# neoyinyao/Recommender

Measured on AMD Instinct MI355X. Metric: examples/sec fwd+bwd, Criteo-DLRM 26×40M×128 batch 65536, 1/2/4/8 GPU, higher is better.
Workload: dtype fp32; 1 GPU; dlrm_criteo_26x40000000x128; global_batch=65536, per_gpu_batch=65536, rows=40000000, dim=128, slots=26, optimizer=sgd, parallelism=single, prefetch=False

## Files before the change

recommender_amd/csrc/sort.hip:

```cpp
#include "common.hpp"

namespace rs {

constexpr int kSortThreads = 256;
constexpr int kSortKeysPerLane = 16;
constexpr int kSortTile = kSortThreads * kSortKeysPerLane;
constexpr int kSortKeysPerLaneSmall = 4;
constexpr int kSortKeysPerLaneTiny = 2;
constexpr int64_t kSortSmallN = 1 << 20;
constexpr int64_t kSortTinyN = 1 << 17;
static inline int sort_kpl(int64_t n) {
  return n < kSortTinyN ? kSortKeysPerLaneTiny : (n < kSortSmallN ? kSortKeysPerLaneSmall : kSortKeysPerLane);
}
constexpr int kMaxBins = 512;

template <int BITS>
__device__ __forceinline__ uint64_t match_digit(uint32_t digit, bool valid) {
  uint32_t mis_lo = 0u, mis_hi = 0u;
#pragma unroll
  for (int b = 0; b < BITS; ++b) {
    const uint32_t sgn = (uint32_t)(-(int32_t)((digit >> b) & 1u));
    const uint64_t bb = __ballot(sgn != 0u);
    mis_lo |= (uint32_t)bb ^ sgn;
    mis_hi |= (uint32_t)(bb >> 32) ^ sgn;
// ... 338 lines not shown
    flags[i] = (k < key_space && (i == 0 || keys[i - 1] != k)) ? 1 : 0;
  }
}

__global__ void unique_inverse_kernel(const uint32_t* __restrict__ keys, const int32_t* __restrict__ pos,
                                      const int32_t* __restrict__ excl, int64_t n, uint32_t key_space,
                                      uint32_t* __restrict__ uniq, int32_t* __restrict__ inverse) {
  int64_t i = blockIdx.x * (int64_t)blockDim.x + threadIdx.x;
  int64_t stride = (int64_t)gridDim.x * blockDim.x;
  for (; i < n; i += stride) {
    const uint32_t k = keys[i];
    const bool valid = k < key_space;
    const bool head = valid && (i == 0 || keys[i - 1] != k);
    const int32_t seg = excl[i] + (head ? 1 : 0) - 1;
    if (head) uniq[seg] = k;
    inverse[pos[i]] = valid ? seg : -1;
  }
}

__global__ void owner_counts_kernel(const uint32_t* __restrict__ uniq, const int32_t* __restrict__ n_unique,
                                    int64_t shard_stride, int32_t world, int32_t* __restrict__ counts) {
  const int o = threadIdx.x;
  if (o >= world) return;
  const int32_t nu = *n_unique;
  auto lb = [&](int64_t v) {
    int32_t lo = 0, hi = nu;
    while (lo < hi) {
      int32_t mid = (lo + hi) >> 1;
      if ((int64_t)uniq[mid] < v) lo = mid + 1; else hi = mid;
    }
    return lo;
  };
  counts[o] = lb((int64_t)(o + 1) * shard_stride) - lb((int64_t)o * shard_stride);
}

static int key_bits_for(int64_t n_rows) {
  int b = 1;
  while (b < 32 && ((int64_t)1 << b) <= n_rows) ++b;
  return b;
}

struct SortPlan {
  int passes;
  int bits;
  int kpl;
  int n_tiles;
};

static SortPlan plan_sort(int64_t n_ids, int64_t n_rows) {
  SortPlan p;
  int kb = key_bits_for(n_rows);
  p.passes = (kb + 8) / 9;
  p.bits = (kb + p.passes - 1) / p.passes;
  p.kpl = sort_kpl(n_ids);
  p.n_tiles = (int)ceil_div(n_ids, (int64_t)kSortThreads * p.kpl);
  return p;
}

static size_t sort_ws_layout(int64_t n_ids, Carver& c, uint32_t** keys_alt, int32_t** vals_alt,
                             int32_t** hist, int32_t** totals) {
  int n_tiles = (int)ceil_div(n_ids, (int64_t)kSortThreads * sort_kpl(n_ids));
  *keys_alt = c.take<uint32_t>(n_ids);
  *vals_alt = c.take<int32_t>(n_ids);
  *hist = c.take<int32_t>((size_t)kMaxBins * n_tiles + 1);
  *totals = c.take<int32_t>(kMaxBins);
  return c.off;
}

template <int BITS, bool FIRST_FROM_IDS, int KPL>
static int32_t launch_pass_k(uint32_t* kin, const int32_t* vin, uint32_t* kout, int32_t* vout,
                             int64_t n, int shift, int32_t* hist, int32_t* totals, int n_tiles,
                             const KeyGen& kg, hipStream_t st, uint32_t clamp_key) {
  radix_hist_kernel<BITS, FIRST_FROM_IDS, KPL><<<n_tiles, kSortThreads, 0, st>>>(kin, kg, n, shift,
                                                                                 hist, n_tiles);
  RS_CHECK_LAUNCH();
  constexpr int BINS = 1 << BITS;
  radix_colscan_kernel<<<(BINS + 3) / 4, 256, 0, st>>>(hist, n_tiles, BINS, totals);
  RS_CHECK_LAUNCH();
  radix_scatter_kernel<BITS, FIRST_FROM_IDS, KPL><<<n_tiles, kSortThreads, 0, st>>>(
      kin, vin, n, shift, hist, totals, n_tiles, kout, vout, clamp_key);
  RS_CHECK_LAUNCH();
  return RS_OK;
}

template <int BITS, bool FIRST_FROM_IDS>
static int32_t launch_pass(uint32_t* kin, const int32_t* vin, uint32_t* kout, int32_t* vout,
                           int64_t n, int shift, int32_t* hist, int32_t* totals, int n_tiles,
                           const KeyGen& kg, hipStream_t st, uint32_t clamp_key) {
  if (sort_kpl(n) == kSortKeysPerLaneTiny)
    return launch_pass_k<BITS, FIRST_FROM_IDS, kSortKeysPerLaneTiny>(kin, vin, kout, vout, n, shift,
                                                                     hist, totals, n_tiles, kg, st,
                                                                     clamp_key);
  if (sort_kpl(n) == kSortKeysPerLaneSmall)
    return launch_pass_k<BITS, FIRST_FROM_IDS, kSortKeysPerLaneSmall>(kin, vin, kout, vout, n, shift,
                                                                      hist, totals, n_tiles, kg, st,
                                                                      clamp_key);
  return launch_pass_k<BITS, FIRST_FROM_IDS, kSortKeysPerLane>(kin, vin, kout, vout, n, shift, hist,
                                                               totals, n_tiles, kg, st, clamp_key);
}

template <bool FIRST_FROM_IDS>
static int32_t dispatch_pass(int bits, uint32_t* kin, const int32_t* vin, uint32_t* kout,
                             int32_t* vout, int64_t n, int shift, int32_t* hist, int32_t* totals,
                             int n_tiles, const KeyGen& kg, hipStream_t st, uint32_t clamp_key) {
#define RS_PASS(B) \
  case B: return launch_pass<B, FIRST_FROM_IDS>(kin, vin, kout, vout, n, shift, hist, totals, n_tiles, kg, st, clamp_key);
  switch (bits) {
    RS_PASS(1) RS_PASS(2) RS_PASS(3) RS_PASS(4) RS_PASS(5) RS_PASS(6) RS_PASS(7) RS_PASS(8) RS_PASS(9)
  }
#undef RS_PASS
  set_error("radix pass bits %d unsupported", bits);
  return RS_E_UNSUPPORTED;
}

static int32_t radix_sort_impl(uint32_t* keys_in, int32_t* vals_in, uint32_t* keys_out,
                               int32_t* vals_out, int64_t n, int64_t max_key, void* ws,
                               size_t ws_bytes, const KeyGen* kg, hipStream_t st) {
  SortPlan p = plan_sort(n, max_key);
  Carver c(ws, ws_bytes);
  uint32_t* kalt;
  int32_t* valt;
  int32_t* hist;
  int32_t* totals;
  sort_ws_layout(n, c, &kalt, &valt, &hist, &totals);
  if (!c.ok()) {
    set_error("sort workspace too small: need %zu have %zu", c.off, ws_bytes);
    return RS_E_WORKSPACE;
  }
  uint32_t* ka = keys_in;
  int32_t* va = vals_in;
  const KeyGen none{};
  for (int pass = 0; pass < p.passes; ++pass) {
    bool last = pass == p.passes - 1;
    uint32_t* kb = last ? keys_out : (ka == keys_in ? kalt : keys_in);
    int32_t* vb = last ? vals_out : (va == vals_in ? valt : vals_in);
    const uint32_t clamp = (last && kg) ? static_cast<uint32_t>(kg->key_space) : 0xFFFFFFFFu;
    int32_t s = (pass == 0 && kg)
                    ? dispatch_pass<true>(p.bits, ka, va, kb, vb, n, 0, hist, totals, p.n_tiles, *kg, st,
                                          clamp)
                    : dispatch_pass<false>(p.bits, ka, va, kb, vb, n, pass * p.bits, hist, totals,
                                           p.n_tiles, none, st, clamp);
    if (s) return s;
    ka = kb;
    va = vb;
  }
  return RS_OK;
}

int32_t radix_sort_pairs(uint32_t* keys_in, int32_t* vals_in, uint32_t* keys_out,
                         int32_t* vals_out, int64_t n, int64_t n_rows, void* ws, size_t ws_bytes,
                         hipStream_t st) {
  return radix_sort_impl(keys_in, vals_in, keys_out, vals_out, n, n_rows, ws, ws_bytes, nullptr, st);
}

size_t radix_sort_ws_size(int64_t n) {
  Carver c(nullptr, 0);
  uint32_t* a;
  int32_t* b;
  int32_t* h;
  int32_t* t;
  return sort_ws_layout(n, c, &a, &b, &h, &t) + 256;
}

__global__ __launch_bounds__(1024) void scan_single_block_kernel(int32_t* __restrict__ a, int64_t n,
                                                                 int32_t* __restrict__ total) {
  __shared__ int32_t wsum[16];
  __shared__ int32_t carry_s;
  const int t = threadIdx.x, lane = t & 63, w = t >> 6;
  if (t == 0) carry_s = 0;
  __syncthreads();
  for (int64_t base = 0; base < n; base += 4096) {
    int32_t v[4];
    int64_t i0 = base + (int64_t)t * 4;
#pragma unroll
    for (int k = 0; k < 4; ++k) v[k] = (i0 + k < n) ? a[i0 + k] : 0;
    int32_t s = v[0] + v[1] + v[2] + v[3];
    int32_t x = s;
#pragma unroll
    for (int off = 1; off < 64; off <<= 1) {
      int32_t y = __shfl_up(x, off);
      if (lane >= off) x += y;
    }
    if (lane == 63) wsum[w] = x;
    __syncthreads();
    if (t < 16) {
      int32_t ws = wsum[t];
      int32_t xs = ws;
#pragma unroll
      for (int off = 1; off < 16; off <<= 1) {
        int32_t y = __shfl_up(xs, off, 16);
        if ((t & 15) >= off) xs += y;
      }
      wsum[t] = xs - ws;
    }
    __syncthreads();
    int32_t run = carry_s + wsum[w] + x - s;
#pragma unroll
    for (int k = 0; k < 4; ++k) {
      if (i0 + k < n) a[i0 + k] = run;
      run += v[k];
    }
    __syncthreads();
    if (t == 1023) carry_s = run;
    __syncthreads();
  }
  if (t == 0 && total) *total = carry_s;
}

constexpr int kScanThreads = 256;
constexpr int kScanPerThread = 16;
constexpr int kScanTile = kScanThreads * kScanPerThread;

__global__ __launch_bounds__(kScanThreads) void scan_tile_sums_kernel(const int32_t* __restrict__ in,
                                                                      int64_t n,
                                                                      int32_t* __restrict__ sums) {
  __shared__ int32_t red[kScanThreads / 64];
  int64_t base = (int64_t)blockIdx.x * kScanTile;
  int32_t s = 0;
  int32_t v[kScanPerThread];
#pragma unroll
  for (int k = 0; k < kScanPerThread; ++k) {
    const int64_t i = base + (int64_t)k * kScanThreads + threadIdx.x;
    v[k] = in[i < n ? i : 0];
  }
#pragma unroll
  for (int k = 0; k < kScanPerThread; ++k)
    if (base + (int64_t)k * kScanThreads + threadIdx.x < n) s += v[k];
  for (int off = 32; off > 0; off >>= 1) s += __shfl_down(s, off);
  if ((threadIdx.x & 63) == 0) red[threadIdx.x >> 6] = s;
  __syncthreads();
  if (threadIdx.x == 0) {
    int32_t t = 0;
    for (int w = 0; w < kScanThreads / 64; ++w) t += red[w];
    sums[blockIdx.x] = t;
  }
}

__global__ __launch_bounds__(kScanThreads) void scan_tile_apply_kernel(const int32_t* __restrict__ in,
                                                                       int64_t n,
                                                                       const int32_t* __restrict__ sums,
                                                                       int32_t* __restrict__ out) {
  __shared__ int32_t part[kScanThreads];
  int64_t base = (int64_t)blockIdx.x * kScanTile + (int64_t)threadIdx.x * kScanPerThread;
  int32_t v[kScanPerThread];
  int32_t s = 0;
#pragma unroll
  for (int k = 0; k < kScanPerThread; ++k) {
    int64_t i = base + k;
    v[k] = i < n ? in[i] : 0;
    s += v[k];
  }
  part[threadIdx.x] = s;
  __syncthreads();
  for (int off = 1; off < kScanThreads; off <<= 1) {
    int32_t t = threadIdx.x >= off ? part[threadIdx.x - off] : 0;
    __syncthreads();
    part[threadIdx.x] += t;
    __syncthreads();
  }
  int32_t run = sums[blockIdx.x] + (threadIdx.x ? part[threadIdx.x - 1] : 0);
#pragma unroll
  for (int k = 0; k < kScanPerThread; ++k) {
    int64_t i = base + k;
    if (i < n) out[i] = run;
    run += v[k];
  }
}

size_t exclusive_scan_ws_size(int64_t n) { return align_up((ceil_div(n, kScanTile) + 1) * 4, 256); }

int32_t exclusive_scan_i32(const int32_t* in, int32_t* out, int64_t n, int32_t* total, void* ws,
                           size_t ws_bytes, hipStream_t st) {
  int64_t tiles = ceil_div(n, kScanTile);
  if (ws_bytes < exclusive_scan_ws_size(n)) {
    set_error("scan workspace too small");
    return RS_E_WORKSPACE;
  }
  int32_t* sums = static_cast<int32_t*>(ws);
  if (n == 0) {
    if (total) RS_CHECK_HIP(hipMemsetAsync(total, 0, 4, st));
    return RS_OK;
  }
  scan_tile_sums_kernel<<<tiles, kScanThreads, 0, st>>>(in, n, sums);
  RS_CHECK_LAUNCH();
  scan_single_block_kernel<<<1, 1024, 0, st>>>(sums, tiles, total);
  RS_CHECK_LAUNCH();
  scan_tile_apply_kernel<<<tiles, kScanThreads, 0, st>>>(in, n, sums, out);
  RS_CHECK_LAUNCH();
  return RS_OK;
}

constexpr int kSegThreads = 256;
#ifndef RS_SEG_KPL
#define RS_SEG_KPL 16
#endif
constexpr int kSegKPL = RS_SEG_KPL;
constexpr int kSegTile = kSegThreads * kSegKPL;
constexpr int kSegBits = 12;
constexpr int kSegBins = 1 << kSegBits;
constexpr int kSegMaxTiles = 32 * 16 / kSegKPL;
constexpr int kSegMaxSlots = 64;
constexpr int kSegMaxBits = 2 * kSegBits;
constexpr int kNumXcd = 8;

struct SegArgs {
  const void* ids;
  int32_t dtype;
  const uint8_t* valid;
  const int64_t* slot_offsets;
  int n_slots;
  int64_t B;
  int tiles;
  int64_t n_rows;
  uint16_t* hist0;
  uint16_t* hist1;
  int32_t* vcnt;
  int32_t* scnt;
  uint2* tmp;
  uint32_t* keys0;
  int32_t* starts;
  uint32_t* rows_out;
  int32_t* pos_out;
  int32_t* err_flag;
};

__device__ __forceinline__ int seg_bits(int64_t rows) {
  int b = 0;
  while (b < 31 && ((int64_t)1 << b) < rows) ++b;
  return b;
}

struct SegSlot {
  int64_t lo, rows;
  int w0, w1;
};

__device__ __forceinline__ SegSlot seg_slot(const SegArgs& a, int s) {
  SegSlot r;
  r.lo = a.slot_offsets ? a.slot_offsets[s] : 0;
  r.rows = a.slot_offsets ? a.slot_offsets[s + 1] - r.lo : a.n_rows;
  const int bits = seg_bits(r.rows);
  r.w0 = bits < kSegBits ? bits : kSegBits;
  r.w1 = bits - r.w0;
  if (r.w1 > kSegBits) {
    r.w1 = kSegBits;
    r.rows = (int64_t)1 << kSegMaxBits;
    if (threadIdx.x == 0 && a.err_flag) atomicOr(a.err_flag, RS_ERRBIT_RANGE);
  }
  return r;
}

__device__ __forceinline__ void seg_tile0(const SegArgs& a, int& s, int& t) {
  const int x = blockIdx.x % kNumXcd, rest = blockIdx.x / kNumXcd;
  s = rest % a.n_slots;
  t = (rest / a.n_slots) * kNumXcd + x;
}
__device__ __forceinline__ void seg_tile1(const SegArgs& a, int& s, int& t) {
  const int x = blockIdx.x % kNumXcd, rest = blockIdx.x / kNumXcd;
  const int spx = (a.n_slots + kNumXcd - 1) / kNumXcd;
  s = x + kNumXcd * (rest % spx);
  t = rest / spx;
}

template <bool ID64>
__device__ __forceinline__ void seg_load0(const SegArgs& a, const SegSlot& sl, int s, int t,
                                          uint32_t (&id)[kSegKPL], uint32_t& live,
                                          uint32_t& sent, bool& oob) {
  const int wave = threadIdx.x >> 6, lane = threadIdx.x & 63;
  int64_t v[kSegKPL];
  int64_t pp[kSegKPL];
  uint32_t inb = 0u;
#pragma unroll
  for (int k = 0; k < kSegKPL; ++k) {
    const int64_t b = (int64_t)t * kSegTile + wave * 64 * kSegKPL + k * 64 + lane;
    const bool in = b < a.B;
    inb |= (uint32_t)in << k;
    pp[k] = in ? b * a.n_slots + s : 0;
    v[k] = ID64 ? static_cast<const int64_t*>(a.ids)[pp[k]]
                : static_cast<int64_t>(static_cast<const int32_t*>(a.ids)[pp[k]]);
  }
  uint32_t excl = 0u;
  if (a.valid) {
    uint8_t f[kSegKPL];
#pragma unroll
    for (int k = 0; k < kSegKPL; ++k) f[k] = a.valid[pp[k]];
#pragma unroll
    for (int k = 0; k < kSegKPL; ++k) excl |= (uint32_t)(f[k] == 0) << k;
  }
  live = 0u;
  sent = 0u;
#pragma unroll
  for (int k = 0; k < kSegKPL; ++k) {
    id[k] = 0u;
    if ((inb >> k) & 1u) {
      if ((excl >> k) & 1u) {
        sent |= 1u << k;
      } else if (v[k] < 0 || v[k] >= sl.rows) {
        sent |= 1u << k;
        oob = true;
      } else {
        id[k] = static_cast<uint32_t>(v[k]);
        live |= 1u << k;
      }
    }
  }
}

__device__ __forceinline__ void seg_store_hist(uint16_t* __restrict__ h, const int32_t* cnt, int bins) {
  for (int d = threadIdx.x; d < bins; d += blockDim.x) h[d] = static_cast<uint16_t>(cnt[d]);
}

template <bool ID64>
__global__ __launch_bounds__(kSegThreads) void slot_sort_hist0_kernel(SegArgs a) {
  __shared__ int32_t cnt[kSegBins];
  __shared__ int32_t nsent;
  int s, t;
  seg_tile0(a, s, t);
  if (s >= a.n_slots || t >= a.tiles) return;
  const SegSlot sl = seg_slot(a, s);
  const int bins = 1 << sl.w0;
  for (int d = threadIdx.x; d < bins; d += blockDim.x) cnt[d] = 0;
  if (threadIdx.x == 0) nsent = 0;
  __syncthreads();
  uint32_t id[kSegKPL], live, sent;
  bool oob = false;
  seg_load0<ID64>(a, sl, s, t, id, live, sent, oob);
  const int lane = threadIdx.x & 63;
  const uint32_t mask = (uint32_t)bins - 1u;
  int ns = 0;
#pragma unroll
  for (int k = 0; k < kSegKPL; ++k) {
    if ((live >> k) & 1u) atomicAdd(&cnt[id[k] & mask], 1);
    ns += __popcll(__ballot((sent >> k) & 1u));
  }
  if (lane == 0 && ns) atomicAdd(&nsent, ns);
  if (__any(oob) && lane == 0) flag_oob(a.err_flag);
  const int64_t tile = (int64_t)s * a.tiles + t;
  {
    const int wave = threadIdx.x >> 6;
    uint32_t* kt = a.keys0 + tile * kSegTile + wave * 64 * kSegKPL + lane;
#pragma unroll
    for (int k = 0; k < kSegKPL; ++k) kt[k * 64] = ((sent >> k) & 1u) ? 0x80000000u : id[k];
  }
  __syncthreads();
  seg_store_hist(a.hist0 + tile * kSegBins, cnt, bins);
  if (threadIdx.x == 0) {
    const int64_t b0 = (int64_t)t * kSegTile;
    const int64_t tn = a.B - b0 < kSegTile ? a.B - b0 : kSegTile;
    a.vcnt[tile] = (int32_t)tn - nsent;
    a.scnt[tile] = nsent;
  }
}

__device__ __forceinline__ void seg_slot_starts(const SegArgs& a, int32_t* vstart, int32_t* sstart,
                                                int s, int t, int32_t* spre) {
  if (threadIdx.x <= a.n_slots) {
    vstart[threadIdx.x] = 0;
    sstart[threadIdx.x] = 0;
  }
  if (threadIdx.x == 0) *spre = 0;
  __syncthreads();
  constexpr int kPer = kSegMaxSlots * kSegMaxTiles / kSegThreads;
  const int total = a.n_slots * a.tiles;
  int32_t cv[kPer], cz[kPer];
#pragma unroll
  for (int i = 0; i < kPer; ++i) {
    const int e = threadIdx.x + i * kSegThreads;
    const int ec = e < total ? e : 0;
    cv[i] = a.vcnt[ec];
    cz[i] = a.scnt[ec];
  }
  int32_t mine = 0;
#pragma unroll
  for (int i = 0; i < kPer; ++i) {
    const int e = threadIdx.x + i * kSegThreads;
    if (e < total) {
      const int sl = e / a.tiles;
      if (cv[i]) atomicAdd(&vstart[sl], cv[i]);
      if (cz[i]) atomicAdd(&sstart[sl], cz[i]);
      if (sl == s && e - sl * a.tiles < t) mine += cz[i];
    }
  }
  if (mine) atomicAdd(spre, mine);
  __syncthreads();
  if (threadIdx.x < 64) {
    const int lane = threadIdx.x;
    const int32_t v = lane < a.n_slots ? vstart[lane] : 0, z = lane < a.n_slots ? sstart[lane] : 0;
    int32_t xv = v, xz = z;
#pragma unroll
    for (int off = 1; off < 64; off <<= 1) {
      const int32_t yv = __shfl_up(xv, off), yz = __shfl_up(xz, off);
      if (lane >= off) {
        xv += yv;
        xz += yz;
      }
    }
    if (lane < a.n_slots) {
      vstart[lane] = xv - v;
      sstart[lane] = xz - z;
    }
    if (lane == 63) {
      vstart[a.n_slots] = xv;
      sstart[a.n_slots] = xz;
    }
  }
  __syncthreads();
}

__device__ __forceinline__ void seg_rank(const uint32_t (&dig)[kSegKPL], uint32_t live,
                                         uint16_t (*wcnt)[kSegBins], int bins,
                                         int32_t (&rank)[kSegKPL]) {
  const int wave = threadIdx.x >> 6, lane = threadIdx.x & 63;
  const uint64_t lt = lanemask_lt64();
  for (int e = threadIdx.x; e < 4 * bins; e += blockDim.x) wcnt[e / bins][e % bins] = 0;
  __syncthreads();
#pragma unroll
  for (int k = 0; k < kSegKPL; ++k) {
    const bool lv = (live >> k) & 1u;
    const uint32_t d = dig[k];
    const uint64_t m = match_digit<kSegBits>(d, lv);
    const int32_t before = __popcll(m & lt);
    const int32_t prev = lv ? wcnt[wave][d] : 0;
    rank[k] = prev + before;
    __builtin_amdgcn_wave_barrier();
    if (lv && (m >> lane) == 1ull) wcnt[wave][d] = (uint16_t)(prev + before + 1);
    __builtin_amdgcn_wave_barrier();
  }
  __syncthreads();
  for (int d = threadIdx.x; d < bins; d += blockDim.x) {
    int32_t run = 0;
#pragma unroll
    for (int w = 0; w < 4; ++w) {
      const int32_t c = wcnt[w][d];
      wcnt[w][d] = (uint16_t)run;
      run += c;
    }
  }
  __syncthreads();
}

__device__ __forceinline__ void seg_offsets_inblock(const uint16_t* __restrict__ hist, int n_tiles,
                                                    int t, int bins, int32_t base,
                                                    int32_t* __restrict__ doff, int32_t* wsum) {
  constexpr int PER = kSegBins / kSegThreads;
  const int d0 = threadIdx.x * PER;
  int32_t tot[PER], pre[PER];
#pragma unroll
  for (int i = 0; i < PER; ++i) tot[i] = pre[i] = 0;
  if (d0 < bins) {
    constexpr int kBatch = 8;
    for (int u0 = 0; u0 < n_tiles; u0 += kBatch) {
      uint4 q[kBatch][2];
#pragma unroll
      for (int j = 0; j < kBatch; ++j) {
        const int u = u0 + j < n_tiles ? u0 + j : 0;
        const uint4* row = reinterpret_cast<const uint4*>(hist + (int64_t)u * kSegBins + d0);
        q[j][0] = row[0];
        q[j][1] = row[1];
      }
#pragma unroll
      for (int j = 0; j < kBatch; ++j) {
        const int u = u0 + j;
        if (u < n_tiles) {
          const uint32_t w[8] = {q[j][0].x, q[j][0].y, q[j][0].z, q[j][0].w,
                                 q[j][1].x, q[j][1].y, q[j][1].z, q[j][1].w};
#pragma unroll
          for (int i = 0; i < PER; ++i) {
            const int32_t c = d0 + i < bins ? (int32_t)((w[i >> 1] >> (16 * (i & 1))) & 0xFFFFu) : 0;
            tot[i] += c;
            if (u < t) pre[i] += c;
          }
        }
      }
    }
  }
  int32_t mine = 0;
#pragma unroll
  for (int i = 0; i < PER; ++i) mine += tot[i];
  const int lane = threadIdx.x & 63, wave = threadIdx.x >> 6;
  int32_t x = mine;
#pragma unroll
  for (int off = 1; off < 64; off <<= 1) {
    const int32_t y = __shfl_up(x, off);
    if (lane >= off) x += y;
  }
  if (lane == 63) wsum[wave] = x;
  __syncthreads();
  int32_t run = base + x - mine;
  for (int w = 0; w < wave; ++w) run += wsum[w];
  if (d0 < bins) {
#pragma unroll
    for (int i = 0; i < PER; ++i) {
      if (d0 + i < bins) doff[d0 + i] = run + pre[i];
      run += tot[i];
    }
  }
  __syncthreads();
}

template <bool ID64>
__global__ __launch_bounds__(kSegThreads) void slot_sort_scatter0_kernel(SegArgs a) {
  __shared__ uint16_t wcnt[4][kSegBins];
  __shared__ int32_t doff[kSegBins];
  __shared__ int32_t wsent[4];
  int s, t;
  seg_tile0(a, s, t);
  if (s >= a.n_slots || t >= a.tiles) return;
  const SegSlot sl = seg_slot(a, s);
  const int bins = 1 << sl.w0;
  uint32_t id[kSegKPL], live = 0u, sent = 0u;
  {
    const int64_t b0 = (int64_t)t * kSegTile;
    const int tn = (int)(a.B - b0 < kSegTile ? a.B - b0 : kSegTile);
    const int w0 = (threadIdx.x >> 6) * 64 * kSegKPL + (threadIdx.x & 63);
    const uint32_t* kt = a.keys0 + ((int64_t)s * a.tiles + t) * kSegTile + w0;
    uint32_t raw[kSegKPL];
#pragma unroll
    for (int k = 0; k < kSegKPL; ++k) raw[k] = kt[k * 64];
#pragma unroll
    for (int k = 0; k < kSegKPL; ++k) {
      const bool in = w0 + k * 64 < tn;
      const uint32_t v = in ? raw[k] : 0u;
      id[k] = v & 0x7FFFFFFFu;
      if (in && (v >> 31)) sent |= 1u << k;
      else if (in) live |= 1u << k;
    }
  }
  __shared__ int32_t vstart[kSegMaxSlots + 1], sstart[kSegMaxSlots + 1], wsc[4], spre_sh;
  seg_slot_starts(a, vstart, sstart, s, t, &spre_sh);
  if (s == 0 && t == 0)
    for (int q = threadIdx.x; q <= a.n_slots; q += blockDim.x) {
      a.starts[q] = vstart[q];
      a.starts[kSegMaxSlots + 1 + q] = sstart[q];
    }
  const int32_t spre = spre_sh;
  seg_offsets_inblock(a.hist0 + (int64_t)s * a.tiles * kSegBins, a.tiles, t, bins, vstart[s], doff,
                      wsc);
  const int32_t n_valid = vstart[a.n_slots];
  const int32_t sent_base = n_valid + sstart[s] + spre;
  uint32_t dig[kSegKPL];
  const uint32_t mask = (uint32_t)bins - 1u;
#pragma unroll
  for (int k = 0; k < kSegKPL; ++k) dig[k] = id[k] & mask;
  int32_t rank[kSegKPL];
  seg_rank(dig, live, wcnt, bins, rank);
  const int wave = threadIdx.x >> 6, lane = threadIdx.x & 63;
  const uint64_t lt = lanemask_lt64();
  int32_t srank[kSegKPL];
  int32_t srun = 0;
#pragma unroll
  for (int k = 0; k < kSegKPL; ++k) {
    const uint64_t m = __ballot((sent >> k) & 1u);
    srank[k] = srun + __popcll(m & lt);
    srun += __popcll(m);
  }
  if (lane == 0) wsent[wave] = srun;
  __syncthreads();
  int32_t sbase = sent_base;
  for (int w = 0; w < wave; ++w) sbase += wsent[w];
  const bool final_pass = sl.w1 == 0;
#pragma unroll
  for (int k = 0; k < kSegKPL; ++k) {
    const int64_t b = (int64_t)t * kSegTile + wave * 64 * kSegKPL + k * 64 + lane;
    const int32_t p = (int32_t)(b * a.n_slots + s);
    if ((live >> k) & 1u) {
      const int32_t dst = doff[dig[k]] + wcnt[wave][dig[k]] + rank[k];
      if (final_pass) {
        a.rows_out[dst] = static_cast<uint32_t>(sl.lo + id[k]);
        a.pos_out[dst] = p;
      } else {
        a.tmp[dst] = make_uint2(id[k], static_cast<uint32_t>(p));
      }
    } else if ((sent >> k) & 1u) {
      const int32_t dst = sbase + srank[k];
      a.rows_out[dst] = static_cast<uint32_t>(a.n_rows);
      a.pos_out[dst] = p;
    }
  }
}

__device__ __forceinline__ void seg_load1(const SegArgs& a, int32_t start, int32_t n_s, int t,
                                          uint32_t (&id)[kSegKPL], int32_t (&pos)[kSegKPL],
                                          uint32_t& live) {
  const int wave = threadIdx.x >> 6, lane = threadIdx.x & 63;
  live = 0u;
#pragma unroll
  for (int k = 0; k < kSegKPL; ++k) {
    const int32_t j = t * kSegTile + wave * 64 * kSegKPL + k * 64 + lane;
    id[k] = 0u;
    pos[k] = 0;
    if (j < n_s) {
      const uint2 e = a.tmp[start + j];
      id[k] = e.x;
      pos[k] = static_cast<int32_t>(e.y);
      live |= 1u << k;
    }
  }
}

__global__ __launch_bounds__(kSegThreads) void slot_sort_hist1_kernel(SegArgs a) {
  __shared__ int32_t cnt[kSegBins];
  int s, t;
  seg_tile1(a, s, t);
  if (s >= a.n_slots || t >= a.tiles) return;
  const SegSlot sl = seg_slot(a, s);
  if (sl.w1 == 0) return;
  const int32_t start = a.starts[s], n_s = a.starts[s + 1] - start;
  if (t * kSegTile >= n_s) return;
  const int bins = 1 << sl.w1;
  uint32_t id[kSegKPL], live;
  int32_t pos[kSegKPL];
  seg_load1(a, start, n_s, t, id, pos, live);
  for (int d = threadIdx.x; d < bins; d += blockDim.x) cnt[d] = 0;
  __syncthreads();
#pragma unroll
  for (int k = 0; k < kSegKPL; ++k)
    if ((live >> k) & 1u) atomicAdd(&cnt[id[k] >> sl.w0], 1);
  __syncthreads();
  seg_store_hist(a.hist1 + ((int64_t)s * a.tiles + t) * kSegBins, cnt, bins);
}

__global__ __launch_bounds__(kSegThreads) void slot_sort_scatter1_kernel(SegArgs a) {
  __shared__ uint16_t wcnt[4][kSegBins];
  __shared__ int32_t doff[kSegBins];
  int s, t;
  seg_tile1(a, s, t);
  if (s >= a.n_slots || t >= a.tiles) return;
  const SegSlot sl = seg_slot(a, s);
  if (sl.w1 == 0) return;
  const int32_t start = a.starts[s], n_s = a.starts[s + 1] - start;
  if (t * kSegTile >= n_s) return;
  const int bins = 1 << sl.w1;
  uint32_t id[kSegKPL], live;
  int32_t pos[kSegKPL];
  seg_load1(a, start, n_s, t, id, pos, live);
  __shared__ int32_t wsc[4];
  seg_offsets_inblock(a.hist1 + (int64_t)s * a.tiles * kSegBins, (n_s + kSegTile - 1) / kSegTile,
                      t, bins, start, doff, wsc);
  uint32_t dig[kSegKPL];
#pragma unroll
  for (int k = 0; k < kSegKPL; ++k) dig[k] = id[k] >> sl.w0;
  int32_t rank[kSegKPL];
  seg_rank(dig, live, wcnt, bins, rank);
  const int wave = threadIdx.x >> 6;
#pragma unroll
  for (int k = 0; k < kSegKPL; ++k) {
    if ((live >> k) & 1u) {
      const int32_t dst = doff[dig[k]] + wcnt[wave][dig[k]] + rank[k];
      a.rows_out[dst] = static_cast<uint32_t>(sl.lo + id[k]);
      a.pos_out[dst] = pos[k];
    }
  }
}

constexpr int kSmallThreads = 1024, kSmallWaves = kSmallThreads / 64;
constexpr int kSmallMax = 16384, kSmallKPT = kSmallMax / kSmallThreads;
constexpr int kSmallPosBits = 14;
constexpr int64_t kSmallMaxRows = (int64_t(1) << (32 - kSmallPosBits)) - 2;
constexpr int kSmallDigitMax = 9, kSmallBins = 1 << kSmallDigitMax;

template <bool BOUNDED>
__global__ __launch_bounds__(kSmallThreads) void small_sort_kernel(
    const void* __restrict__ ids, int32_t dtype, int64_t n, const uint8_t* __restrict__ valid,
    const int64_t* __restrict__ slot_offsets, int64_t n_rows, int key_bits,
    uint32_t* __restrict__ rows_out, int32_t* __restrict__ pos_out, int32_t* __restrict__ n_unique,
    int32_t* __restrict__ err_flag) {
  __shared__ uint32_t bufs[2][kSmallMax];
  __shared__ uint16_t wcnt[kSmallWaves][kSmallBins];
  __shared__ int32_t dbase[kSmallBins];
  __shared__ int32_t heads[kSmallWaves];
  const int wave = threadIdx.x >> 6, lane = threadIdx.x & 63;
  const uint64_t lt = lanemask_lt64();
  const int64_t lo = slot_offsets ? slot_offsets[0] : 0;
  const int64_t span = slot_offsets ? slot_offsets[1] - lo : n_rows;
  const int own = wave * (kSmallKPT * 64) + lane;
  bool oob = false;
#pragma unroll 4
  for (int r = 0; r < kSmallKPT; ++r) {
    const int i = own + r * 64;
    uint32_t e = 0xFFFFFFFFu;
    if (i < n) {
      uint32_t key = (uint32_t)n_rows;
      if (!valid || valid[i]) {
        const int64_t id = load_id(ids, dtype, i);
        if (id >= 0 && id < span) key = (uint32_t)(lo + id);
        else oob = true;
      }
      e = key << kSmallPosBits | (uint32_t)i;
    }
    bufs[0][i] = e;
  }
  if (__any(oob) && lane == 0) flag_oob(err_flag);
  const int passes = (key_bits + kSmallDigitMax - 1) / kSmallDigitMax;
  const int per = (key_bits + passes - 1) / passes;
  int cur = 0;
  for (int shift = kSmallPosBits; shift < kSmallPosBits + key_bits; shift += per) {
    const int nb = kSmallPosBits + key_bits - shift < per ? kSmallPosBits + key_bits - shift : per;
    const int bins = 1 << nb;
    const uint32_t dmask = (uint32_t)bins - 1u;
    const uint32_t* src = bufs[cur];
    uint32_t* dst = bufs[cur ^ 1];
    for (int e = threadIdx.x; e < kSmallWaves * kSmallBins; e += kSmallThreads) (&wcnt[0][0])[e] = 0;
    __syncthreads();
    uint32_t ent[kSmallKPT];
    int32_t rank[kSmallKPT];
#pragma unroll
    for (int r = 0; r < kSmallKPT; ++r) {
      ent[r] = 0u;
      rank[r] = 0;
      if (!BOUNDED || wave * (kSmallKPT * 64) + r * 64 < n) {
        const bool in = !BOUNDED || own + r * 64 < n;
        ent[r] = src[own + r * 64];
        const uint32_t d = (ent[r] >> shift) & dmask;
        const uint64_t m = match_digit_n<kSmallDigitMax>(d, in, nb);
        const int32_t prev = in ? wcnt[wave][d] : 0;
        rank[r] = prev + __popcll(m & lt);
        __builtin_amdgcn_wave_barrier();
        if (in && (m >> lane) == 1ull) wcnt[wave][d] = (uint16_t)(prev + __popcll(m));
        __builtin_amdgcn_wave_barrier();
      }
    }
    __syncthreads();
    if (threadIdx.x < bins) {
      const int d = threadIdx.x;
      int32_t run = 0;
#pragma unroll
      for (int w = 0; w < kSmallWaves; ++w) {
        const int32_t c = wcnt[w][d];
        wcnt[w][d] = (uint16_t)run;
        run += c;
      }
      dbase[d] = run;
    }
    __syncthreads();
    if (threadIdx.x < 64) {
      constexpr int Q = kSmallBins / 64;
      int32_t t[Q], sum = 0;
#pragma unroll
      for (int q = 0; q < Q; ++q) {
        t[q] = Q * lane + q < bins ? dbase[Q * lane + q] : 0;
        sum += t[q];
      }
      int32_t x = sum;
#pragma unroll
      for (int off = 1; off < 64; off <<= 1) {
        const int32_t y = __shfl_up(x, off);
        if (lane >= off) x += y;
      }
      int32_t run = x - sum;
#pragma unroll
      for (int q = 0; q < Q; ++q) {
        if (Q * lane + q < bins) dbase[Q * lane + q] = run;
        run += t[q];
      }
    }
    __syncthreads();
#pragma unroll
    for (int r = 0; r < kSmallKPT; ++r) {
      if (!BOUNDED || own + r * 64 < n) {
        const uint32_t d = (ent[r] >> shift) & dmask;
        dst[dbase[d] + wcnt[wave][d] + rank[r]] = ent[r];
      }
    }
    __syncthreads();
    cur ^= 1;
  }
  const uint32_t* out = bufs[cur];
  int32_t h = 0;
  for (int i = threadIdx.x; i < n; i += kSmallThreads) {
    const uint32_t e = out[i];
    const uint32_t key = e >> kSmallPosBits;
    rows_out[i] = key;
    pos_out[i] = (int32_t)(e & ((1u << kSmallPosBits) - 1u));
    if (key < (uint32_t)n_rows && (i == 0 || (out[i - 1] >> kSmallPosBits) != key)) ++h;
  }
  if (n_unique) {
#pragma unroll
    for (int off = 32; off > 0; off >>= 1) h += __shfl_xor(h, off);
    if (lane == 0) heads[wave] = h;
    __syncthreads();
    if (threadIdx.x == 0) {
      int32_t t = 0;
      for (int w = 0; w < kSmallWaves; ++w) t += heads[w];
      *n_unique = t;
    }
  }
}

constexpr int kMaxRuns = 1024;

__global__ __launch_bounds__(256) void runs_merge_kernel(const int32_t* __restrict__ ids, int64_t n,
                                                         int n_runs, int64_t run_len,
                                                         int64_t n_rows, uint32_t* __restrict__ rows_out,
                                                         int32_t* __restrict__ pos_out,
                                                         int32_t* __restrict__ err_flag) {
  __shared__ int64_t vl[kMaxRuns];
  __shared__ int64_t padb[kMaxRuns];
  __shared__ int64_t nvalid;
  for (int r = threadIdx.x; r < n_runs; r += blockDim.x) {
    const int32_t* run = ids + (int64_t)r * run_len;
    int64_t lo = 0, hi = run_len;
    while (lo < hi) {
      const int64_t mid = (lo + hi) >> 1;
      const int32_t v = run[mid];
      if (v >= 0 && v < n_rows) lo = mid + 1;
      else hi = mid;
    }
    vl[r] = lo;
  }
  __syncthreads();
  if (threadIdx.x == 0) {
    int64_t acc = 0, pad = 0;
    for (int r = 0; r < n_runs; ++r) {
      padb[r] = pad;
      acc += vl[r];
      pad += run_len - vl[r];
    }
    nvalid = acc;
  }
  __syncthreads();
  bool oob = false;
  for (int64_t e = blockIdx.x * (int64_t)blockDim.x + threadIdx.x; e < n;
       e += (int64_t)gridDim.x * blockDim.x) {
    const int s = (int)(e / run_len);
    const int64_t j = e - (int64_t)s * run_len;
    const int32_t key = ids[e];
    int64_t out;
    uint32_t kout;
    if (j < vl[s]) {
      out = j;
      for (int r = 0; r < n_runs; ++r) {
        if (r == s) continue;
        const int32_t* run = ids + (int64_t)r * run_len;
        int64_t lo = 0, hi = vl[r];
        if (r < s) {
          while (lo < hi) {
            const int64_t mid = (lo + hi) >> 1;
            if (run[mid] <= key) lo = mid + 1; else hi = mid;
          }
        } else {
          while (lo < hi) {
            const int64_t mid = (lo + hi) >> 1;
            if (run[mid] < key) lo = mid + 1; else hi = mid;
          }
        }
        out += lo;
      }
      kout = (uint32_t)key;
    } else {
      out = nvalid + padb[s] + (j - vl[s]);
      kout = (uint32_t)n_rows;
      if (key >= n_rows) oob = true;
    }
    rows_out[out] = kout;
    pos_out[out] = (int32_t)e;
  }
  flag_oob_wave(oob, err_flag);
}

static bool small_eligible(int64_t n_ids, int n_slots, int world, int64_t n_rows) {
  return world == 1 && n_slots == 1 && n_ids >= 1 && n_ids <= kSmallMax && n_rows <= kSmallMaxRows;
}

static int32_t small_sort(const void* ids, int32_t id_dtype, int64_t n_ids, const uint8_t* valid,
                          const int64_t* slot_offsets, int64_t n_rows, uint32_t* sorted_rows,
                          int32_t* sorted_pos, int32_t* n_unique, int32_t* err_flag, hipStream_t st) {
  int key_bits = 1;
  while (key_bits < 32 - kSmallPosBits && (int64_t(1) << key_bits) <= n_rows) ++key_bits;
  if (n_ids <= kSmallMax * 3 / 4)
    small_sort_kernel<true><<<1, kSmallThreads, 0, st>>>(ids, id_dtype, n_ids, valid, slot_offsets,
                                                          n_rows, key_bits, sorted_rows, sorted_pos,
                                                          n_unique, err_flag);
  else
    small_sort_kernel<false><<<1, kSmallThreads, 0, st>>>(ids, id_dtype, n_ids, valid, slot_offsets, n_rows,
                                                 key_bits, sorted_rows, sorted_pos, n_unique,
                                                 err_flag);
  RS_CHECK_LAUNCH();
  return RS_OK;
}

static size_t seg_ws_layout(int64_t n, int n_slots, int tiles, Carver& c, SegArgs* a) {
  const size_t nt = (size_t)n_slots * tiles;
  uint32_t* k0 = c.take<uint32_t>(nt * kSegTile);
  uint16_t* h0 = c.take<uint16_t>(nt * kSegBins);
  uint16_t* h1 = c.take<uint16_t>(nt * kSegBins);
  int32_t* v = c.take<int32_t>(nt);
  int32_t* z = c.take<int32_t>(nt);
  int32_t* st = c.take<int32_t>(2 * (kSegMaxSlots + 1));
  uint2* tmp = c.take<uint2>(n);
  if (a) {
    a->keys0 = k0;
    a->hist0 = h0;
    a->hist1 = h1;
    a->vcnt = v;
    a->scnt = z;
    a->starts = st;
    a->tmp = tmp;
  }
  return c.off;
}

static bool seg_eligible(int64_t n_ids, int n_slots, int world, int64_t max_slot_rows) {
  if (world != 1 || n_slots < 1 || n_slots > kSegMaxSlots || n_ids < 1) return false;
  if (n_ids % n_slots) return false;
  const int64_t B = n_ids / n_slots;
  return B <= (int64_t)kSegMaxTiles * kSegTile && max_slot_rows >= 1 &&
         max_slot_rows <= ((int64_t)1 << kSegMaxBits);
}

size_t seg_ws_size(int64_t n_ids) {
  const int64_t tiles_total = n_ids / kSegTile + kSegMaxSlots;
  Carver c(nullptr, 0);
  return seg_ws_layout(n_ids, 1, (int)tiles_total, c, nullptr) + 1024;
}

static int32_t seg_sort(const void* ids, int32_t id_dtype, int64_t n_ids, const uint8_t* valid,
                        const int64_t* slot_offsets, int n_slots, int64_t n_rows,
                        uint32_t* sorted_rows, int32_t* sorted_pos, int32_t* err_flag,
                        void* workspace, size_t ws_bytes, hipStream_t st) {
  SegArgs a{};
  a.ids = ids;
  a.dtype = id_dtype;
  a.valid = valid;
  a.slot_offsets = slot_offsets;
  a.n_slots = n_slots;
  a.B = n_ids / n_slots;
  a.tiles = (int)ceil_div(a.B, kSegTile);
  a.n_rows = n_rows;
  a.rows_out = sorted_rows;
  a.pos_out = sorted_pos;
  a.err_flag = err_flag;
  Carver c(workspace, ws_bytes);
  seg_ws_layout(n_ids, n_slots, a.tiles, c, &a);
  if (!c.ok()) {
    set_error("sort workspace too small: need %zu have %zu", c.off, ws_bytes);
    return RS_E_WORKSPACE;
  }
  const int tiles_pad = (int)ceil_div(a.tiles, kNumXcd) * kNumXcd;
  const int grid0 = tiles_pad * n_slots;
  const int spx = (int)ceil_div(n_slots, kNumXcd);
  const int grid1 = kNumXcd * spx * a.tiles;
  if (id_dtype == RS_ID_I64) slot_sort_hist0_kernel<true><<<grid0, kSegThreads, 0, st>>>(a);
  else slot_sort_hist0_kernel<false><<<grid0, kSegThreads, 0, st>>>(a);
  RS_CHECK_LAUNCH();
  if (id_dtype == RS_ID_I64) slot_sort_scatter0_kernel<true><<<grid0, kSegThreads, 0, st>>>(a);
  else slot_sort_scatter0_kernel<false><<<grid0, kSegThreads, 0, st>>>(a);
  RS_CHECK_LAUNCH();
  slot_sort_hist1_kernel<<<grid1, kSegThreads, 0, st>>>(a);
  RS_CHECK_LAUNCH();
  slot_sort_scatter1_kernel<<<grid1, kSegThreads, 0, st>>>(a);
  RS_CHECK_LAUNCH();
  return RS_OK;
}
// ... 189 lines not shown
```

Baseline: 105.0 million examples/sec.

## Cut register pressure in segmented radix sort by processing keys in halves

The segmented slot-sort kernels now handle their per-lane keys in two halves, with loops kept rolled. Ranks are packed two per 32-bit register, and keys are reloaded from global memory between the ranking and scatter phases instead of staying live in registers. Launch bounds now request 8 blocks per CU, and the offset-scan batch drops from 8 to 2, all to lower VGPR usage and raise occupancy. The cost is extra global reloads of keys and tmp entries, plus less instruction-level parallelism from the rolled loops.

```diff
diff --git a/recommender_amd/csrc/sort.hip b/recommender_amd/csrc/sort.hip
--- a/recommender_amd/csrc/sort.hip
+++ b/recommender_amd/csrc/sort.hip
@@ -664,6 +664,9 @@
 constexpr int kSegMaxSlots = 64;
 constexpr int kSegMaxBits = 2 * kSegBits;
 constexpr int kNumXcd = 8;
+#define RS_SEG_KERNEL __launch_bounds__(kSegThreads, 8)
+constexpr int kSegHalf = kSegKPL / 2;
+static_assert(kSegKPL % 2 == 0 && 64 * kSegKPL <= 65536, "two halves; wave ranks fit 16 bits");
 
 struct SegArgs {
   const void* ids;
@@ -725,36 +728,36 @@
 }
 
 template <bool ID64>
-__device__ __forceinline__ void seg_load0(const SegArgs& a, const SegSlot& sl, int s, int t,
-                                          uint32_t (&id)[kSegKPL], uint32_t& live,
+__device__ __forceinline__ void seg_load0(const SegArgs& a, const SegSlot& sl, int s, int t, int h,
+                                          uint32_t (&id)[kSegHalf], uint32_t& live,
                                           uint32_t& sent, bool& oob) {
   const int wave = threadIdx.x >> 6, lane = threadIdx.x & 63;
-  int64_t v[kSegKPL];
-  int64_t pp[kSegKPL];
-  uint32_t inb = 0u;
-#pragma unroll
-  for (int k = 0; k < kSegKPL; ++k) {
-    const int64_t b = (int64_t)t * kSegTile + wave * 64 * kSegKPL + k * 64 + lane;
-    const bool in = b < a.B;
-    inb |= (uint32_t)in << k;
-    pp[k] = in ? b * a.n_slots + s : 0;
-    v[k] = ID64 ? static_cast<const int64_t*>(a.ids)[pp[k]]
-                : static_cast<int64_t>(static_cast<const int32_t*>(a.ids)[pp[k]]);
+  const int64_t b0 = (int64_t)t * kSegTile + wave * 64 * kSegKPL + h * kSegHalf * 64 + lane;
+  auto pos_of = [&](int k) -> int64_t {
+    const int64_t b = b0 + k * 64;
+    return b < a.B ? b * a.n_slots + s : 0;
+  };
+  int64_t v[kSegHalf];
+#pragma unroll
+  for (int k = 0; k < kSegHalf; ++k) {
+    const int64_t p = pos_of(k);
+    v[k] = ID64 ? static_cast<const int64_t*>(a.ids)[p]
+                : static_cast<int64_t>(static_cast<const int32_t*>(a.ids)[p]);
   }
   uint32_t excl = 0u;
   if (a.valid) {
-    uint8_t f[kSegKPL];
-#pragma unroll
-    for (int k = 0; k < kSegKPL; ++k) f[k] = a.valid[pp[k]];
-#pragma unroll
-    for (int k = 0; k < kSegKPL; ++k) excl |= (uint32_t)(f[k] == 0) << k;
+    uint8_t f[kSegHalf];
+#pragma unroll
+    for (int k = 0; k < kSegHalf; ++k) f[k] = a.valid[pos_of(k)];
+#pragma unroll
+    for (int k = 0; k < kSegHalf; ++k) excl |= (uint32_t)(f[k] == 0) << k;
   }
   live = 0u;
   sent = 0u;
 #pragma unroll
-  for (int k = 0; k < kSegKPL; ++k) {
+  for (int k = 0; k < kSegHalf; ++k) {
     id[k] = 0u;
-    if ((inb >> k) & 1u) {
+    if (b0 + k * 64 < a.B) {
       if ((excl >> k) & 1u) {
         sent |= 1u << k;
       } else if (v[k] < 0 || v[k] >= sl.rows) {
@@ -773,7 +776,7 @@
 }
 
 template <bool ID64>
-__global__ __launch_bounds__(kSegThreads) void slot_sort_hist0_kernel(SegArgs a) {
+__global__ RS_SEG_KERNEL void slot_sort_hist0_kernel(SegArgs a) {
   __shared__ int32_t cnt[kSegBins];
   __shared__ int32_t nsent;
   int s, t;
@@ -784,26 +787,26 @@
   for (int d = threadIdx.x; d < bins; d += blockDim.x) cnt[d] = 0;
   if (threadIdx.x == 0) nsent = 0;
   __syncthreads();
-  uint32_t id[kSegKPL], live, sent;
+  const int wave = threadIdx.x >> 6, lane = threadIdx.x & 63;
+  const uint32_t mask = (uint32_t)bins - 1u;
+  const int64_t tile = (int64_t)s * a.tiles + t;
   bool oob = false;
-  seg_load0<ID64>(a, sl, s, t, id, live, sent, oob);
-  const int lane = threadIdx.x & 63;
-  const uint32_t mask = (uint32_t)bins - 1u;
   int ns = 0;
-#pragma unroll
-  for (int k = 0; k < kSegKPL; ++k) {
-    if ((live >> k) & 1u) atomicAdd(&cnt[id[k] & mask], 1);
-    ns += __popcll(__ballot((sent >> k) & 1u));
+#pragma unroll 1
+  for (int h = 0; h < 2; ++h) {
+    uint32_t id[kSegHalf], live, sent;
+    seg_load0<ID64>(a, sl, s, t, h, id, live, sent, oob);
+#pragma unroll
+    for (int k = 0; k < kSegHalf; ++k) {
+      if ((live >> k) & 1u) atomicAdd(&cnt[id[k] & mask], 1);
+      ns += __popcll(__ballot((sent >> k) & 1u));
+    }
+    uint32_t* kt = a.keys0 + tile * kSegTile + wave * 64 * kSegKPL + h * kSegHalf * 64 + lane;
+#pragma unroll
+    for (int k = 0; k < kSegHalf; ++k) kt[k * 64] = ((sent >> k) & 1u) ? 0x80000000u : id[k];
   }
   if (lane == 0 && ns) atomicAdd(&nsent, ns);
   if (__any(oob) && lane == 0) flag_oob(a.err_flag);
-  const int64_t tile = (int64_t)s * a.tiles + t;
-  {
-    const int wave = threadIdx.x >> 6;
-    uint32_t* kt = a.keys0 + tile * kSegTile + wave * 64 * kSegKPL + lane;
-#pragma unroll
-    for (int k = 0; k < kSegKPL; ++k) kt[k * 64] = ((sent >> k) & 1u) ? 0x80000000u : id[k];
-  }
   __syncthreads();
   seg_store_hist(a.hist0 + tile * kSegBins, cnt, bins);
   if (threadIdx.x == 0) {
@@ -869,25 +872,23 @@
   __syncthreads();
 }
 
-__device__ __forceinline__ void seg_rank(const uint32_t (&dig)[kSegKPL], uint32_t live,
-                                         uint16_t (*wcnt)[kSegBins], int bins,
-                                         int32_t (&rank)[kSegKPL]) {
-  const int wave = threadIdx.x >> 6, lane = threadIdx.x & 63;
-  const uint64_t lt = lanemask_lt64();
+__device__ __forceinline__ void seg_rank_begin(uint16_t (*wcnt)[kSegBins], int bins) {
   for (int e = threadIdx.x; e < 4 * bins; e += blockDim.x) wcnt[e / bins][e % bins] = 0;
   __syncthreads();
-#pragma unroll
-  for (int k = 0; k < kSegKPL; ++k) {
-    const bool lv = (live >> k) & 1u;
-    const uint32_t d = dig[k];
-    const uint64_t m = match_digit<kSegBits>(d, lv);
-    const int32_t before = __popcll(m & lt);
-    const int32_t prev = lv ? wcnt[wave][d] : 0;
-    rank[k] = prev + before;
-    __builtin_amdgcn_wave_barrier();
-    if (lv && (m >> lane) == 1ull) wcnt[wave][d] = (uint16_t)(prev + before + 1);
-    __builtin_amdgcn_wave_barrier();
-  }
+}
+
+__device__ __forceinline__ uint32_t seg_rank_key(uint32_t d, bool lv, uint16_t* wcnt_wave) {
+  const int lane = threadIdx.x & 63;
+  const uint64_t m = match_digit<kSegBits>(d, lv);
+  const int32_t before = __popcll(m & lanemask_lt64());
+  const int32_t prev = lv ? wcnt_wave[d] : 0;
+  __builtin_amdgcn_wave_barrier();
+  if (lv && (m >> lane) == 1ull) wcnt_wave[d] = (uint16_t)(prev + before + 1);
+  __builtin_amdgcn_wave_barrier();
+  return (uint32_t)(prev + before);
+}
+
+__device__ __forceinline__ void seg_rank_end(uint16_t (*wcnt)[kSegBins], int bins) {
   __syncthreads();
   for (int d = threadIdx.x; d < bins; d += blockDim.x) {
     int32_t run = 0;
@@ -910,7 +911,8 @@
 #pragma unroll
   for (int i = 0; i < PER; ++i) tot[i] = pre[i] = 0;
   if (d0 < bins) {
-    constexpr int kBatch = 8;
+    constexpr int kBatch = 2;
+#pragma unroll 1
     for (int u0 = 0; u0 < n_tiles; u0 += kBatch) {
       uint4 q[kBatch][2];
 #pragma unroll
@@ -960,8 +962,26 @@
   __syncthreads();
 }
 
+__device__ __forceinline__ void seg_keys0(const uint32_t* __restrict__ kt, int w0, int tn, int h,
+                                          uint32_t (&id)[kSegHalf], uint32_t& live,
+                                          uint32_t& sent) {
+  uint32_t raw[kSegHalf];
+#pragma unroll
+  for (int k = 0; k < kSegHalf; ++k) raw[k] = kt[(h * kSegHalf + k) * 64];
+  live = 0u;
+  sent = 0u;
+#pragma unroll
+  for (int k = 0; k < kSegHalf; ++k) {
+    const bool in = w0 + (h * kSegHalf + k) * 64 < tn;
+    const uint32_t v = in ? raw[k] : 0u;
+    id[k] = v & 0x7FFFFFFFu;
+    if (in && (v >> 31)) sent |= 1u << k;
+    else if (in) live |= 1u << k;
+  }
+}
+
 template <bool ID64>
-__global__ __launch_bounds__(kSegThreads) void slot_sort_scatter0_kernel(SegArgs a) {
+__global__ RS_SEG_KERNEL void slot_sort_scatter0_kernel(SegArgs a) {
   __shared__ uint16_t wcnt[4][kSegBins];
   __shared__ int32_t doff[kSegBins];
   __shared__ int32_t wsent[4];
@@ -970,24 +990,6 @@
   if (s >= a.n_slots || t >= a.tiles) return;
   const SegSlot sl = seg_slot(a, s);
   const int bins = 1 << sl.w0;
-  uint32_t id[kSegKPL], live = 0u, sent = 0u;
-  {
-    const int64_t b0 = (int64_t)t * kSegTile;
-    const int tn = (int)(a.B - b0 < kSegTile ? a.B - b0 : kSegTile);
-    const int w0 = (threadIdx.x >> 6) * 64 * kSegKPL + (threadIdx.x & 63);
-    const uint32_t* kt = a.keys0 + ((int64_t)s * a.tiles + t) * kSegTile + w0;
-    uint32_t raw[kSegKPL];
-#pragma unroll
-    for (int k = 0; k < kSegKPL; ++k) raw[k] = kt[k * 64];
-#pragma unroll
-    for (int k = 0; k < kSegKPL; ++k) {
-      const bool in = w0 + k * 64 < tn;
-      const uint32_t v = in ? raw[k] : 0u;
-      id[k] = v & 0x7FFFFFFFu;
-      if (in && (v >> 31)) sent |= 1u << k;
-      else if (in) live |= 1u << k;
-    }
-  }
   __shared__ int32_t vstart[kSegMaxSlots + 1], sstart[kSegMaxSlots + 1], wsc[4], spre_sh;
   seg_slot_starts(a, vstart, sstart, s, t, &spre_sh);
   if (s == 0 && t == 0)
@@ -1000,67 +1002,87 @@
                       wsc);
   const int32_t n_valid = vstart[a.n_slots];
   const int32_t sent_base = n_valid + sstart[s] + spre;
-  uint32_t dig[kSegKPL];
   const uint32_t mask = (uint32_t)bins - 1u;
-#pragma unroll
-  for (int k = 0; k < kSegKPL; ++k) dig[k] = id[k] & mask;
-  int32_t rank[kSegKPL];
-  seg_rank(dig, live, wcnt, bins, rank);
   const int wave = threadIdx.x >> 6, lane = threadIdx.x & 63;
   const uint64_t lt = lanemask_lt64();
-  int32_t srank[kSegKPL];
+  const int64_t b0 = (int64_t)t * kSegTile;
+  const int tn = (int)(a.B - b0 < kSegTile ? a.B - b0 : kSegTile);
+  const int w0 = wave * 64 * kSegKPL + lane;
+  const uint32_t* kt = a.keys0 + ((int64_t)s * a.tiles + t) * kSegTile + w0;
+  uint32_t rk[kSegHalf];
+#pragma unroll
+  for (int k = 0; k < kSegHalf; ++k) rk[k] = 0u;
+  seg_rank_begin(wcnt, bins);
   int32_t srun = 0;
-#pragma unroll
-  for (int k = 0; k < kSegKPL; ++k) {
-    const uint64_t m = __ballot((sent >> k) & 1u);
-    srank[k] = srun + __popcll(m & lt);
-    srun += __popcll(m);
+#pragma unroll 1
+  for (int h = 0; h < 2; ++h) {
+    uint32_t id[kSegHalf], live, sent;
+    seg_keys0(kt, w0, tn, h, id, live, sent);
+#pragma unroll
+    for (int k = 0; k < kSegHalf; ++k) {
+      rk[k] |= seg_rank_key(id[k] & mask, (live >> k) & 1u, wcnt[wave]) << (16 * h);
+      srun += __popcll(__ballot((sent >> k) & 1u));
+    }
   }
   if (lane == 0) wsent[wave] = srun;
-  __syncthreads();
+  seg_rank_end(wcnt, bins);
   int32_t sbase = sent_base;
   for (int w = 0; w < wave; ++w) sbase += wsent[w];
   const bool final_pass = sl.w1 == 0;
-#pragma unroll
-  for (int k = 0; k < kSegKPL; ++k) {
-    const int64_t b = (int64_t)t * kSegTile + wave * 64 * kSegKPL + k * 64 + lane;
-    const int32_t p = (int32_t)(b * a.n_slots + s);
-    if ((live >> k) & 1u) {
-      const int32_t dst = doff[dig[k]] + wcnt[wave][dig[k]] + rank[k];
-      if (final_pass) {
-        a.rows_out[dst] = static_cast<uint32_t>(sl.lo + id[k]);
+#pragma unroll 1
+  for (int h = 0; h < 2; ++h) {
+    uint32_t id[kSegHalf], live, sent;
+    seg_keys0(kt, w0, tn, h, id, live, sent);
+#pragma unroll
+    for (int k = 0; k < kSegHalf; ++k) {
+      const int64_t b = b0 + w0 + (h * kSegHalf + k) * 64;
+      const int32_t p = (int32_t)(b * a.n_slots + s);
+      const uint64_t m = __ballot((sent >> k) & 1u);
+      if ((live >> k) & 1u) {
+        const uint32_t d = id[k] & mask;
+        const int32_t dst = doff[d] + wcnt[wave][d] + (int32_t)((rk[k] >> (16 * h)) & 0xFFFFu);
+        if (final_pass) {
+          a.rows_out[dst] = static_cast<uint32_t>(sl.lo + id[k]);
+          a.pos_out[dst] = p;
+        } else {
+          a.tmp[dst] = make_uint2(id[k], static_cast<uint32_t>(p));
+        }
+      } else if ((sent >> k) & 1u) {
+        const int32_t dst = sbase + __popcll(m & lt);
+        a.rows_out[dst] = static_cast<uint32_t>(a.n_rows);
         a.pos_out[dst] = p;
-      } else {
-        a.tmp[dst] = make_uint2(id[k], static_cast<uint32_t>(p));
-      }
-    } else if ((sent >> k) & 1u) {
-      const int32_t dst = sbase + srank[k];
-      a.rows_out[dst] = static_cast<uint32_t>(a.n_rows);
-      a.pos_out[dst] = p;
+      }
+      sbase += __popcll(m);
     }
   }
 }
 
 __device__ __forceinline__ void seg_load1(const SegArgs& a, int32_t start, int32_t n_s, int t,
-                                          uint32_t (&id)[kSegKPL], int32_t (&pos)[kSegKPL],
-                                          uint32_t& live) {
+                                          int h, uint2 (&e)[kSegHalf], uint32_t& live) {
   const int wave = threadIdx.x >> 6, lane = threadIdx.x & 63;
+  const int32_t j0 = t * kSegTile + wave * 64 * kSegKPL + h * kSegHalf * 64 + lane;
   live = 0u;
 #pragma unroll
-  for (int k = 0; k < kSegKPL; ++k) {
-    const int32_t j = t * kSegTile + wave * 64 * kSegKPL + k * 64 + lane;
-    id[k] = 0u;
-    pos[k] = 0;
-    if (j < n_s) {
-      const uint2 e = a.tmp[start + j];
-      id[k] = e.x;
-      pos[k] = static_cast<int32_t>(e.y);
-      live |= 1u << k;
-    }
-  }
-}
-
-__global__ __launch_bounds__(kSegThreads) void slot_sort_hist1_kernel(SegArgs a) {
+  for (int k = 0; k < kSegHalf; ++k) {
+    const int32_t j = j0 + k * 64;
+    e[k] = a.tmp[start + (j < n_s ? j : 0)];
+    if (j < n_s) live |= 1u << k;
+  }
+}
+__device__ __forceinline__ void seg_load1_ids(const SegArgs& a, int32_t start, int32_t n_s, int t,
+                                              int h, uint32_t (&id)[kSegHalf], uint32_t& live) {
+  const int wave = threadIdx.x >> 6, lane = threadIdx.x & 63;
+  const int32_t j0 = t * kSegTile + wave * 64 * kSegKPL + h * kSegHalf * 64 + lane;
+  live = 0u;
+#pragma unroll
+  for (int k = 0; k < kSegHalf; ++k) {
+    const int32_t j = j0 + k * 64;
+    id[k] = a.tmp[start + (j < n_s ? j : 0)].x;
+    if (j < n_s) live |= 1u << k;
+  }
+}
+
+__global__ RS_SEG_KERNEL void slot_sort_hist1_kernel(SegArgs a) {
   __shared__ int32_t cnt[kSegBins];
   int s, t;
   seg_tile1(a, s, t);
@@ -1070,19 +1092,21 @@
   const int32_t start = a.starts[s], n_s = a.starts[s + 1] - start;
   if (t * kSegTile >= n_s) return;
   const int bins = 1 << sl.w1;
-  uint32_t id[kSegKPL], live;
-  int32_t pos[kSegKPL];
-  seg_load1(a, start, n_s, t, id, pos, live);
   for (int d = threadIdx.x; d < bins; d += blockDim.x) cnt[d] = 0;
   __syncthreads();
-#pragma unroll
-  for (int k = 0; k < kSegKPL; ++k)
-    if ((live >> k) & 1u) atomicAdd(&cnt[id[k] >> sl.w0], 1);
+#pragma unroll 1
+  for (int h = 0; h < 2; ++h) {
+    uint32_t id[kSegHalf], live;
+    seg_load1_ids(a, start, n_s, t, h, id, live);
+#pragma unroll
+    for (int k = 0; k < kSegHalf; ++k)
+      if ((live >> k) & 1u) atomicAdd(&cnt[id[k] >> sl.w0], 1);
+  }
   __syncthreads();
   seg_store_hist(a.hist1 + ((int64_t)s * a.tiles + t) * kSegBins, cnt, bins);
 }
 
-__global__ __launch_bounds__(kSegThreads) void slot_sort_scatter1_kernel(SegArgs a) {
+__global__ RS_SEG_KERNEL void slot_sort_scatter1_kernel(SegArgs a) {
   __shared__ uint16_t wcnt[4][kSegBins];
   __shared__ int32_t doff[kSegBins];
   int s, t;
@@ -1093,24 +1117,36 @@
   const int32_t start = a.starts[s], n_s = a.starts[s + 1] - start;
   if (t * kSegTile >= n_s) return;
   const int bins = 1 << sl.w1;
-  uint32_t id[kSegKPL], live;
-  int32_t pos[kSegKPL];
-  seg_load1(a, start, n_s, t, id, pos, live);
   __shared__ int32_t wsc[4];
   seg_offsets_inblock(a.hist1 + (int64_t)s * a.tiles * kSegBins, (n_s + kSegTile - 1) / kSegTile,
                       t, bins, start, doff, wsc);
-  uint32_t dig[kSegKPL];
-#pragma unroll
-  for (int k = 0; k < kSegKPL; ++k) dig[k] = id[k] >> sl.w0;
-  int32_t rank[kSegKPL];
-  seg_rank(dig, live, wcnt, bins, rank);
   const int wave = threadIdx.x >> 6;
-#pragma unroll
-  for (int k = 0; k < kSegKPL; ++k) {
-    if ((live >> k) & 1u) {
-      const int32_t dst = doff[dig[k]] + wcnt[wave][dig[k]] + rank[k];
-      a.rows_out[dst] = static_cast<uint32_t>(sl.lo + id[k]);
-      a.pos_out[dst] = pos[k];
+  uint32_t rk[kSegHalf];
+#pragma unroll
+  for (int k = 0; k < kSegHalf; ++k) rk[k] = 0u;
+  seg_rank_begin(wcnt, bins);
+#pragma unroll 1
+  for (int h = 0; h < 2; ++h) {
+    uint32_t id[kSegHalf], live;
+    seg_load1_ids(a, start, n_s, t, h, id, live);
+#pragma unroll
+    for (int k = 0; k < kSegHalf; ++k)
+      rk[k] |= seg_rank_key(id[k] >> sl.w0, (live >> k) & 1u, wcnt[wave]) << (16 * h);
+  }
+  seg_rank_end(wcnt, bins);
+#pragma unroll 1
+  for (int h = 0; h < 2; ++h) {
+    uint2 e[kSegHalf];
+    uint32_t live;
+    seg_load1(a, start, n_s, t, h, e, live);
+#pragma unroll
+    for (int k = 0; k < kSegHalf; ++k) {
+      if ((live >> k) & 1u) {
+        const uint32_t d = e[k].x >> sl.w0;
+        const int32_t dst = doff[d] + wcnt[wave][d] + (int32_t)((rk[k] >> (16 * h)) & 0xFFFFu);
+        a.rows_out[dst] = static_cast<uint32_t>(sl.lo + e[k].x);
+        a.pos_out[dst] = static_cast<int32_t>(e[k].y);
+      }
     }
   }
 }
```

Measured after the change: 104.9 million examples/sec. No clear change (-0.2%).
